# DeepRec-AI/HybridBackend

Measured on AMD Instinct MI355X. Metric: M-lookups/sec, 26-col Criteo-shape dim16, 1/2/4/8 GPUs; % HBM roofline, higher is better.
Workload: dtype f32

## Files before the change

hybridbackend_amd/csrc/lookup_bwd.hip:

```cpp
#include <alloca.h>
#include <stdlib.h>
#include <string.h>

#include <algorithm>
#include <map>
#include <type_traits>
#include <mutex>
#include <vector>

#include "lookup_common.h"

#ifndef HBK_BWD_WAVES
#define HBK_BWD_WAVES 4
#endif

namespace hbk {
size_t det_sort_temp_bytes(size_t n, int end_bit);
int det_sort_pairs(void* temp, size_t temp_bytes, const uint64_t* keys_in, uint64_t* keys_out,
                   const uint32_t* vals_in, uint32_t* vals_out, size_t n, int end_bit,
                   hipStream_t stream);
size_t det_scan_temp_bytes(size_t n);
int det_scan(void* temp, size_t temp_bytes, const int32_t* in, int32_t* out, size_t n,
             hipStream_t stream);
namespace {
// ... 116 lines not shown
  int64_t n_seg;
  int32_t dim;
  int32_t chunks;
  uint8_t lpr_log2, ids64, combiner, vec4;
  int32_t n_buckets;
  int32_t tile0;
  int32_t bucket0;
  int32_t segtile0;
  int32_t split_t;
  int32_t e_max;
  int32_t merge0;
  int32_t scan0;
  int32_t n_runs;
  int32_t grad_stride;
  uint32_t dense_mul;
  int32_t tpitch;
  uint8_t rowsort;
  uint8_t det;
  uint8_t pad_;
  uint8_t packed;
};

struct GArgs {
  int32_t n_cols;
  float lr;
  int32_t apply;
  int32_t xcd;
  int32_t tile0[kMaxCols];
  int32_t bucket0[kMaxCols];
  int32_t merge0[kMaxCols];
  int32_t scan0[kMaxCols];
  int32_t segtile0[kMaxCols];
  int32_t xcd_w;
  int32_t stage_p;
  int32_t xcd_start[10][9];
  GCol col[kMaxCols];
};
static_assert(sizeof(GArgs) <= 24576, "kernarg budget");
static_assert(kMaxCols <= kWave, "one lane per column in HBK_FIND_COL");
static_assert(kSlots <= 65536 && kCP <= 65536, "16-bit LDS indices");

#define HBK_FIND_COL(ARGS, FIELD)                                                  \
  int ci;                                                                          \
  {                                                                                \
    const int l__ = (int)threadIdx.x & (kWave - 1);                                \
    const int v__ = l__ < (ARGS).n_cols ? (ARGS).FIELD[l__] : 0x7fffffff;          \
    ci = (int)__builtin_popcountll(__ballot(v__ <= (int)blockIdx.x)) - 1;          \
    ci = __builtin_amdgcn_readfirstlane(ci);                                       \
  }                                                                                \
  const auto& c = (ARGS).col[ci];

__device__ inline uint32_t mix32(uint64_t row) {
  uint32_t k = (uint32_t)row ^ ((uint32_t)(row >> 32) * 0x9e3779b1u);
  k ^= k >> 16;
  k *= 0x85ebca6bu;
  k ^= k >> 13;
  k *= 0xc2b2ae35u;
  k ^= k >> 16;
  return k;
}

__device__ inline int bucket_of(const GCol& c, uint64_t row) {
  if (c.dense_mul != 0) return (int)__umulhi((uint32_t)row, c.dense_mul);
  return (int)__umulhi(mix32(row), (uint32_t)c.n_buckets);
}

struct RunCursor {
  int k = -1;
  int64_t next = 0;
  int64_t id_delta = 0;
  int64_t grad_delta = 0;
};

__device__ inline void run_seek(const GCol& c, int64_t j, RunCursor& rc) {
  while (j >= rc.next) {
    ++rc.k;
    const int64_t start = c.run_start[rc.k];
    rc.next = rc.k + 1 < c.n_runs ? c.run_start[rc.k + 1] : (int64_t)1 << 62;
    rc.id_delta = c.run_ids[rc.k] - start;
    rc.grad_delta = c.run_grads[rc.k] - start * c.dim;
  }
}

template <typename V>
__device__ inline void scale_segments(const GCol& c, const float* grad, int32_t stride, int combiner,
                                      int64_t s0, int n, const int32_t* sp) {
  constexpr int VE = sizeof(V) / 4;
  constexpr int kU = 4;
  const int tid = (int)threadIdx.x;
  const int sub = tid & ((1 << c.lpr_log2) - 1);
  const int groups = kBlock >> c.lpr_log2;
  if (sub >= c.chunks) return;
  for (int s = tid >> c.lpr_log2; s < n; s += kU * groups) {
    V g[kU];
    int32_t len[kU];
#pragma unroll
    for (int u = 0; u < kU; ++u) {
      const int ss = s + u * groups < n ? s + u * groups : n - 1;
      len[u] = s + u * groups < n ? sp[ss + 1] - sp[ss] : 0;
      g[u] = __builtin_nontemporal_load(reinterpret_cast<const V*>(
          grad + (s0 + ss) * (int64_t)stride + (int64_t)sub * VE));
    }
#pragma unroll
    for (int u = 0; u < kU; ++u) {
      if (len[u] <= 0) continue;
      const V v = combiner == HBK_COMBINER_MEAN ? g[u] / (float)len[u]
                                                : g[u] / sqrtf((float)len[u]);
      *reinterpret_cast<V*>(c.scaled + (s0 + s + u * groups) * (int64_t)c.dim + (int64_t)sub * VE) = v;
    }
  }
}

__device__ inline int32_t seg_search_wave(const int32_t* splits, int64_t n_seg, int32_t j) {
  const int lane = (int)threadIdx.x & (kWave - 1);
  int64_t lo = 0, n = n_seg;
  while (n > 1) {
    const int64_t step = (n + kWave - 1) / kWave;
    const int64_t s = lo + (int64_t)lane * step;
    const bool le = s < lo + n && splits[s] <= j;
    int k = (int)__builtin_popcountll(__ballot(le));
    if (k < 1) k = 1;
    const int64_t nlo = lo + (int64_t)(k - 1) * step;
    const int64_t rest = lo + n - nlo;
    lo = nlo;
    n = rest < step ? rest : step;
  }
  return (int32_t)lo;
}

__device__ inline int32_t tile_segments(const GCol& c, int64_t j_first, int64_t j_last,
                                        int32_t* seg_lds, int32_t* ends) {
  static_assert(kTile == kBlock * kPerThread && kPerThread % 4 == 0, "whole int4 per thread");
  const int tid = (int)threadIdx.x, lane = tid & (kWave - 1), wave = tid >> 6;
  if (wave == 0) {
    const int32_t s = seg_search_wave(c.splits, c.n_seg, (int32_t)j_first);
    if (tid == 0) ends[0] = s;
  } else if (wave == 1) {
    const int32_t s = seg_search_wave(c.splits, c.n_seg, (int32_t)j_last);
    if (tid == kWave) ends[1] = s;
  }
  int4* const v4 = reinterpret_cast<int4*>(seg_lds) + tid * (kPerThread / 4);
#pragma unroll
  for (int q = 0; q < kPerThread / 4; ++q) v4[q] = make_int4(0, 0, 0, 0);
  __syncthreads();
  const int32_t s_lo = ends[0], s_hi = ends[1];
  for (int32_t s = s_lo + 1 + tid; s <= s_hi; s += kBlock) {
    const int64_t p = (int64_t)c.splits[s] - j_first;
    if (p >= 0 && p < kTile) atomicAdd(&seg_lds[p], 1);
  }
  __syncthreads();
  int32_t x[kPerThread];
#pragma unroll
  for (int q = 0; q < kPerThread / 4; ++q) {
    const int4 v = v4[q];
    x[4 * q] = v.x;
    x[4 * q + 1] = v.y;
    x[4 * q + 2] = v.z;
    x[4 * q + 3] = v.w;
  }
#pragma unroll
  for (int q = 1; q < kPerThread; ++q) x[q] += x[q - 1];
  int32_t incl = x[kPerThread - 1];
#pragma unroll
  for (int o = 1; o < kWave; o <<= 1) {
    const int32_t y = __shfl_up(incl, o, kWave);
    if (lane >= o) incl += y;
  }
  if (lane == kWave - 1) ends[2 + wave] = incl;
  __syncthreads();
  int32_t before = incl - x[kPerThread - 1];
  for (int w = 0; w < wave; ++w) before += ends[2 + w];
#pragma unroll
  for (int q = 0; q < kPerThread / 4; ++q) {
    v4[q] = make_int4(x[4 * q] + before, x[4 * q + 1] + before, x[4 * q + 2] + before,
                      x[4 * q + 3] + before);
  }
  __syncthreads();
  return s_lo;
}

__global__ __launch_bounds__(kBlock) void bwd_segof_kernel(const GArgs a) {
  __shared__ int32_t sp[kBlock + 1];
  HBK_FIND_COL(a, segtile0)
  const int64_t s0 = ((int64_t)blockIdx.x - c.segtile0) * kBlock;
  const int tid = (int)threadIdx.x;
  const int n = c.n_seg - s0 < kBlock ? (int)(c.n_seg - s0) : kBlock;
  if (tid < n) sp[tid] = c.splits[s0 + tid];
  if (tid == 0) sp[n] = c.splits[s0 + n];
  __syncthreads();
  const int32_t lo = sp[0], hi = c.seg_of != nullptr ? sp[n] : sp[0];
  for (int32_t j = lo + tid; j < hi; j += kBlock) {
    int s = 0, e = n;
    while (e - s > 1) {
      const int mid = (s + e) >> 1;
      if (sp[mid] <= j) {
        s = mid;
      } else {
        e = mid;
      }
    }
    c.seg_of[j] = (int32_t)(s0 + s);
  }
  if (c.scaled != nullptr) {
    if (c.vec4) {
      scale_segments<f32x4>(c, c.grad_out, c.grad_stride, c.combiner, s0, n, sp);
    } else {
      scale_segments<float>(c, c.grad_out, c.grad_stride, c.combiner, s0, n, sp);
    }
  }
}

template <bool SIMPLE>
__global__ __launch_bounds__(kBlock) void bwd_hist_kernel(const GArgs a) {
  extern __shared__ int32_t counters[];
  HBK_FIND_COL(a, tile0)
  const int P = c.n_buckets;
  const int tid = (int)threadIdx.x;
  const int ctile = (int)blockIdx.x - c.tile0;
  const int64_t base = (int64_t)ctile * kTile;
  RunCursor rc;
  int64_t id[kBatch];
  auto load_batch = [&](int k0) {
#pragma unroll
    for (int k = 0; k < kBatch; ++k) {
      const int64_t j = base + (int64_t)(k0 + k) * kBlock + tid;
      id[k] = 0;
      if (j < c.n_ids) {
        if (!SIMPLE && c.n_runs > 0) run_seek(c, j, rc);
        id[k] = load_id(c.ids, SIMPLE ? 1 : c.ids64, SIMPLE ? j : j + rc.id_delta);
      }
    }
  };
  load_batch(0);
  for (int p = tid; p < P; p += kBlock) counters[p] = 0;
  __syncthreads();
  for (int k0 = 0; k0 < kPerThread; k0 += kBatch) {
    if (k0 > 0) load_batch(k0);
#pragma unroll
    for (int k = 0; k < kBatch; ++k) {
      const int64_t j = base + (int64_t)(k0 + k) * kBlock + tid;
      if (j < c.n_ids) {
        const uint64_t r = id_to_row(c.map, id[k]);
        if (r != kNoRow) atomicAdd(&counters[SIMPLE ? (int)__umulhi((uint32_t)r, c.dense_mul) : bucket_of(c, r)], 1);
      }
    }
  }
  __syncthreads();
  for (int p = tid; p < P; p += kBlock) c.hist[(int64_t)ctile * P + p] = counters[p];
  if (c.scaled != nullptr) {
    __shared__ int32_t sp[kBlock + 1];
    const int64_t n_tiles = (c.n_ids + kTile - 1) / kTile;
    const int64_t per = (c.n_seg + n_tiles - 1) / n_tiles;
    const int64_t s_begin = (int64_t)ctile * per;
    const int64_t s_end = s_begin + per < c.n_seg ? s_begin + per : c.n_seg;
    for (int64_t s0 = s_begin; s0 < s_end; s0 += kBlock) {
      const int n = s_end - s0 < kBlock ? (int)(s_end - s0) : kBlock;
      __syncthreads();
      if (tid < n) sp[tid] = c.splits[s0 + tid];
      if (tid == 0) sp[n] = c.splits[s0 + n];
      __syncthreads();
      if (c.vec4) {
        scale_segments<f32x4>(c, c.raw_grad, c.raw_stride, c.raw_combiner, s0, n, sp);
      } else {
        scale_segments<float>(c, c.raw_grad, c.raw_stride, c.raw_combiner, s0, n, sp);
      }
    }
  }
}

__device__ inline void scan_tiles_of_bucket(const GCol& c, int p) {
  const int P = c.n_buckets;
  const int n_tiles = (int)((c.n_ids + kTile - 1) / kTile);
  int32_t* h = c.hist + p;
  int32_t run = 0;
  int t = 0;
  for (; t + 16 <= n_tiles; t += 16) {
    int32_t x[16];
#pragma unroll
    for (int k = 0; k < 16; ++k) x[k] = h[(int64_t)(t + k) * P];
#pragma unroll
    for (int k = 0; k < 16; ++k) {
      h[(int64_t)(t + k) * P] = run;
      run += x[k];
    }
  }
  for (; t + 4 <= n_tiles; t += 4) {
    int32_t x[4];
#pragma unroll
    for (int k = 0; k < 4; ++k) x[k] = h[(int64_t)(t + k) * P];
#pragma unroll
    for (int k = 0; k < 4; ++k) {
      h[(int64_t)(t + k) * P] = run;
      run += x[k];
    }
  }
  for (; t < n_tiles; ++t) {
    const int32_t x = h[(int64_t)t * P];
    h[(int64_t)t * P] = run;
    run += x;
  }
  c.bstart[p] = run;
}

__global__ __launch_bounds__(kBlock) void bwd_scan_tiles_kernel(const GArgs a) {
  HBK_FIND_COL(a, scan0)
  const int p = ((int)blockIdx.x - c.scan0) * kBlock + (int)threadIdx.x;
  if (p < c.n_buckets) scan_tiles_of_bucket(c, p);
}

__device__ inline void scan_buckets_of_column(const GCol& c, int32_t* wave_tot, int32_t* n_extra_lds) {
  int32_t& n_extra = *n_extra_lds;
  const int P = c.n_buckets;
  const int tid = (int)threadIdx.x, lane = tid & (kWave - 1), wave = tid >> 6;
  const int per = (P + kBlock - 1) / kBlock;
  const int beg = tid * per;
  const int end = beg + per < P ? beg + per : P;
  if (tid == 0) n_extra = 0;
  int32_t sum = 0;
  for (int p = beg; p < end; ++p) sum += c.bstart[p];
  int32_t incl = sum;
#pragma unroll
  for (int off = 1; off < kWave; off <<= 1) {
    const int32_t y = __shfl_up(incl, off, kWave);
    if (lane >= off) incl += y;
  }
  if (lane == kWave - 1) wave_tot[wave] = incl;
  __syncthreads();
  int32_t run = incl - sum;
  for (int w = 0; w < wave; ++w) run += wave_tot[w];
  for (int p = beg; p < end; ++p) {
    const int32_t n_b = c.bstart[p];
    c.bstart[p] = run;
    c.desc[p] = make_int4(run, n_b, p, 0);
    c.pcount[p] = 0;
    if (n_b > c.split_t) {
      const int32_t extras = (n_b - 1) / c.split_t;
      const int32_t base = atomicAdd(&n_extra, extras);
      for (int32_t e = 0; e < extras; ++e) {
        c.work[2 * (base + e)] = p;
        c.work[2 * (base + e) + 1] = e + 1;
        c.desc[P + base + e] = make_int4(run, n_b, p, e + 1);
      }
    }
    run += n_b;
  }
  __syncthreads();
  for (int e = n_extra + tid; e < c.e_max; e += kBlock) c.desc[P + e] = make_int4(0, 0, -1, 0);
  if (tid == kBlock - 1) {
    c.bstart[P] = run;
    c.counter[0] = 0;
    c.counter[1] = 0;
    *c.n_extra = n_extra;
  }
}

__global__ __launch_bounds__(kBlock) void bwd_scan_kernel(const GArgs a) {
  __shared__ int32_t wave_tot[kWavesPerBlock];
  __shared__ int32_t n_extra;
  scan_buckets_of_column(a.col[blockIdx.x], wave_tot, &n_extra);
}

__global__ __launch_bounds__(kBlock) void bwd_scan_fused_kernel(const GArgs a) {
  __shared__ int32_t wave_tot[kWavesPerBlock];
  __shared__ int32_t n_extra;
  const GCol& c = a.col[blockIdx.x];
  for (int p = (int)threadIdx.x; p < c.n_buckets; p += kBlock) scan_tiles_of_bucket(c, p);
  __syncthreads();
  scan_buckets_of_column(c, wave_tot, &n_extra);
}

constexpr int kXcdScatterBit = 30;

__global__ __launch_bounds__(kBlock) void bwd_scatter_pairs_kernel(const GArgs a) {
  extern __shared__ int32_t run[];
  const int blk = xcd_contiguous((int)blockIdx.x, (int)gridDim.x, (a.xcd >> kXcdScatterBit) & 1);
  int ci;
  {
    const int l__ = (int)threadIdx.x & (kWave - 1);
    const int v__ = l__ < a.n_cols ? a.tile0[l__] : 0x7fffffff;
    ci = (int)__builtin_popcountll(__ballot(v__ <= blk)) - 1;
    ci = __builtin_amdgcn_readfirstlane(ci);
  }
  const GCol& c = a.col[ci];
  const int P = c.n_buckets;
  const int tid = (int)threadIdx.x;
  const int ctile = blk - c.tile0;
  const int64_t base = (int64_t)ctile * kTile;
  __shared__ int32_t sp_lds[kTile];
  __shared__ int32_t seg_ends[2 + kWavesPerBlock];
  const bool seg_inline = c.splits != nullptr && c.seg_of == nullptr;
  int32_t s_lo = 0;
  if (seg_inline) {
    const int64_t j_last = (base + kTile < c.n_ids ? base + kTile : c.n_ids) - 1;
    s_lo = tile_segments(c, base, j_last, sp_lds, seg_ends);
  }
  RunCursor rc;
  int64_t id[kBatch];
  int32_t seg[kBatch];
  auto load_batch = [&](int k0) {
#pragma unroll
    for (int k = 0; k < kBatch; ++k) {
      const int64_t j = base + (int64_t)(k0 + k) * kBlock + tid;
      id[k] = 0;
      seg[k] = (int32_t)j;
      if (j < c.n_ids) {
        if (c.n_runs > 0) {
          run_seek(c, j, rc);
          if (!c.det) seg[k] = (int32_t)(uint32_t)(rc.grad_delta + j * c.dim);
        }
        id[k] = load_id(c.ids, c.ids64, j + rc.id_delta);
        if (c.seg_of != nullptr) {
          seg[k] = c.seg_of[j];
        } else if (seg_inline) {
          seg[k] = s_lo + sp_lds[(k0 + k) * kBlock + tid];
        }
      }
    }
  };
  load_batch(0);
  for (int p = tid; p < P; p += kBlock) run[p] = c.bstart[p] + c.hist[(int64_t)ctile * P + p];
  __syncthreads();
  for (int k0 = 0; k0 < kPerThread; k0 += kBatch) {
    if (k0 > 0) load_batch(k0);
#pragma unroll
    for (int k = 0; k < kBatch; ++k) {
      const int64_t j = base + (int64_t)(k0 + k) * kBlock + tid;
      if (j < c.n_ids) {
        const uint64_t r = id_to_row(c.map, id[k]);
        if (r != kNoRow) {
          const int32_t pos = atomicAdd(&run[bucket_of(c, r)], 1);
          if (c.packed) {
            c.pair_row[0][pos] = (int64_t)((r << 32) | (uint64_t)(uint32_t)seg[k]);
          } else {
            c.pair_row[0][pos] = (int64_t)r;
            c.pair_seg[0][pos] = seg[k];
          }
        }
      }
    }
  }
}

constexpr int kStageMaxBuckets = 1024;

template <bool SIMPLE>
__global__ __launch_bounds__(kBlock, 4) void bwd_scatter_staged_kernel(const GArgs a) {
  extern __shared__ int32_t stage_dyn[];
  int32_t* const counters = stage_dyn;
  int32_t* const first = stage_dyn + a.stage_p;
  int32_t* const st_seg = stage_dyn + 2 * a.stage_p;
  __shared__ int64_t st_row[kTile];
  __shared__ uint16_t st_b[SIMPLE ? 1 : kTile];
  __shared__ int32_t wave_cnt[kWavesPerBlock];
  __shared__ int32_t n_staged;
  const int blk = xcd_contiguous((int)blockIdx.x, (int)gridDim.x, (a.xcd >> kXcdScatterBit) & 1);
  int ci;
  {
    const int l__ = (int)threadIdx.x & (kWave - 1);
    const int v__ = l__ < a.n_cols ? a.tile0[l__] : 0x7fffffff;
    ci = (int)__builtin_popcountll(__ballot(v__ <= blk)) - 1;
    ci = __builtin_amdgcn_readfirstlane(ci);
  }
  const GCol& c = a.col[ci];
  const int P = c.n_buckets;
  const int tid = (int)threadIdx.x, lane = tid & (kWave - 1), wave = tid >> 6;
  const int ctile = blk - c.tile0;
  const int64_t base = (int64_t)ctile * kTile;
  __shared__ int32_t seg_ends[2 + kWavesPerBlock];
  int32_t* const sp_lds = reinterpret_cast<int32_t*>(st_row);
  const bool seg_inline = c.splits != nullptr && (SIMPLE || c.seg_of == nullptr);
  RunCursor rc;
  int64_t id[kPerThread];
  int32_t seg[kPerThread];
#pragma unroll
  for (int k = 0; k < kPerThread; ++k) {
    const int64_t j = base + (int64_t)k * kBlock + tid;
    id[k] = 0;
    seg[k] = (int32_t)j;
    if (j < c.n_ids) {
      if (!SIMPLE && c.n_runs > 0) {
        run_seek(c, j, rc);
        if (!c.det) seg[k] = (int32_t)(uint32_t)(rc.grad_delta + j * c.dim);
      }
      id[k] = load_id(c.ids, SIMPLE ? 1 : c.ids64, SIMPLE ? j : j + rc.id_delta);
      if (!SIMPLE && c.seg_of != nullptr) seg[k] = c.seg_of[j];
    }
  }
  const int per = (P + kBlock - 1) / kBlock;
  const int beg = tid * per;
  const int end = beg + per < P ? beg + per : P;
  int32_t gpos[kStageMaxBuckets / kBlock];
#pragma unroll
  for (int q = 0; q < kStageMaxBuckets / kBlock; ++q) {
    const int p = beg + q;
    gpos[q] = q < per && p < end ? c.bstart[p] + c.hist[(int64_t)ctile * P + p] : 0;
  }
  if (seg_inline) {
    const int64_t j_last = (base + kTile < c.n_ids ? base + kTile : c.n_ids) - 1;
    const int32_t s_lo = tile_segments(c, base, j_last, sp_lds, seg_ends);
#pragma unroll
    for (int k = 0; k < kPerThread; ++k) seg[k] = s_lo + sp_lds[k * kBlock + tid];
  }
  for (int p = tid; p < P; p += kBlock) counters[p] = 0;
  __syncthreads();
  int32_t br[kPerThread];
#pragma unroll
  for (int k = 0; k < kPerThread; ++k) {
    const int64_t j = base + (int64_t)k * kBlock + tid;
    br[k] = -1;
    if (j < c.n_ids) {
      const uint64_t r = id_to_row(c.map, id[k]);
      id[k] = (int64_t)r;
      if (r != kNoRow) {
        const int b = SIMPLE ? (int)__umulhi((uint32_t)r, c.dense_mul) : bucket_of(c, r);
        br[k] = b | (atomicAdd(&counters[b], 1) << 10);
      }
    }
  }
  __syncthreads();
  int32_t sum_c = 0;
#pragma unroll
  for (int q = 0; q < kStageMaxBuckets / kBlock; ++q) {
    if (q < per && beg + q < end) sum_c += counters[beg + q];
  }
  int32_t incl_c = sum_c;
#pragma unroll
  for (int off = 1; off < kWave; off <<= 1) {
    const int32_t w = __shfl_up(incl_c, off, kWave);
    if (lane >= off) incl_c += w;
  }
  if (lane == kWave - 1) wave_cnt[wave] = incl_c;
  __syncthreads();
  int32_t run_c = incl_c - sum_c;
  for (int w = 0; w < wave; ++w) run_c += wave_cnt[w];
#pragma unroll
  for (int q = 0; q < kStageMaxBuckets / kBlock; ++q) {
    const int p = beg + q;
    if (q < per && p < end) {
      const int32_t n_c = counters[p];
      first[p] = run_c;
      counters[p] = gpos[q] - run_c;
      run_c += n_c;
    }
  }
  if (tid == kBlock - 1) n_staged = run_c;
  __syncthreads();
#pragma unroll
  for (int k = 0; k < kPerThread; ++k) {
    if (br[k] >= 0) {
      const int b = br[k] & 1023;
      const int L = first[b] + (br[k] >> 10);
      if (SIMPLE || c.packed) {
        st_row[L] = (int64_t)(((uint64_t)id[k] << 32) | (uint64_t)(uint32_t)seg[k]);
      } else {
        st_row[L] = id[k];
        st_seg[L] = seg[k];
      }
      if (!SIMPLE) st_b[L] = (uint16_t)b;
    }
  }
  __syncthreads();
  const int n_st = n_staged;
#pragma unroll
  for (int k = 0; k < kPerThread; ++k) {
    const int L = k * kBlock + tid;
    if (L < n_st) {
      const int sb = SIMPLE ? (int)__umulhi((uint32_t)((uint64_t)st_row[L] >> 32), c.dense_mul) : (int)st_b[L];
      const int32_t pos = counters[sb] + L;
      c.pair_row[0][pos] = st_row[L];
      if (!SIMPLE && !c.packed) c.pair_seg[0][pos] = st_seg[L];
    }
  }
}

#ifdef HBK_BWD_STAMPS
__device__ unsigned long long g_grp_trace[kTraceBlocks * kTraceSlots];
#define HBK_GSTAMP(i)                                                                       \
  do {                                                                                      \
    if (threadIdx.x == 0 && blockIdx.x < kTraceBlocks) {                                    \
      g_grp_trace[blockIdx.x * kTraceSlots + (i)] = __builtin_amdgcn_s_memrealtime();       \
    }                                                                                       \
  } while (0)
#else
#define HBK_GSTAMP(i)
#endif

constexpr int kGroupMaxBuckets = 2 * kBlock;

struct GSync {
  int32_t* hist;
  int32_t* zero;
  int64_t zero_words;
  SyncWait wait;
};

template <bool SIMPLE>
__global__ __launch_bounds__(kBlock, 4) void bwd_group_kernel(const GArgs a, const GSync y) {
  __shared__ int32_t counters[kGroupMaxBuckets];
  __shared__ int32_t tot_s[kGroupMaxBuckets], pre_s[kGroupMaxBuckets];
  __shared__ int64_t st_row[kTile];
  extern __shared__ int32_t st_seg[];
  __shared__ uint16_t st_b[kTile];
  __shared__ int32_t wave_tot[kWavesPerBlock], wave_cnt[kWavesPerBlock];
  __shared__ int32_t n_extra, gave_up, n_staged;
  const int tid = (int)threadIdx.x, lane = tid & (kWave - 1), wave = tid >> 6;
  HBK_GSTAMP(0);
  for (int64_t j = (int64_t)blockIdx.x * kBlock + tid; j < y.zero_words;
       j += (int64_t)gridDim.x * kBlock) {
    y.zero[j] = 0;
  }
// ... 2425 lines not shown
      if (lr != 0.0f) bits |= (uintptr_t)h.table | (uintptr_t)h.accum | ((uintptr_t)(uint32_t)h.table_pitch * 4);
      vec4 = vec4 && h.dim % 4 == 0 && bits % 16 == 0 && h.n_runs == 0;
      ++k;
    }
    if (k == 0) continue;
    for (int q = k; q <= kMaxCols; ++q) a.base[q] = (int32_t)total;
    a.n_cols = k;
    a.row_bits = bits_for(max_rows);
    a.apply = apply;
    a.lr = lr;
    a.total = total;
    const int end_bit = a.row_bits + (k > 1 ? bits_for((uint64_t)k - 1) : 0);
    a.keys = keys;
    a.vals = vals;
    a.heads = heads;
    a.ranks = ranks;
    hipLaunchKernelGGL(det_keys_kernel, dim3((unsigned)tiles), dim3(kBlock), 0, stream, a);
    HBK_HIP_OK(hipGetLastError());
    int rc = det_sort_pairs(ws + l.temp, l.temp_bytes, keys, skeys, vals, svals, (size_t)total, end_bit,
                            stream);
    if (rc != HBK_OK) return rc;
    a.keys = skeys;
    a.vals = svals;
    const unsigned tiles_p = (unsigned)((total + kDetTile - 1) / kDetTile);
    hipLaunchKernelGGL(det_heads_kernel, dim3(tiles_p), dim3(kBlock), 0, stream, a);
    HBK_HIP_OK(hipGetLastError());
    rc = det_scan(ws + l.temp, l.temp_bytes, heads, ranks, (size_t)total, stream);
    if (rc != HBK_OK) return rc;
    if (vec4) {
      det_launch_reduce<f32x4>(a, max_dim / 4, stream);
    } else {
      det_launch_reduce<float>(a, max_dim, stream);
    }
    HBK_HIP_OK(hipGetLastError());
    hipLaunchKernelGGL(det_counts_kernel, dim3(1), dim3(kWave), 0, stream, a);
    HBK_HIP_OK(hipGetLastError());
  }
  return HBK_OK;
}

}
}

#ifdef HBK_BWD_STAMPS
extern "C" int hbk_debug_grp_trace(unsigned long long* out, int reset) {
  using namespace hbk;
  HBK_HIP_OK(hipDeviceSynchronize());
  if (out != nullptr) {
    HBK_HIP_OK(hipMemcpyFromSymbol(out, HIP_SYMBOL(g_grp_trace), sizeof(g_grp_trace)));
  }
  if (reset) {
    static unsigned long long z[kTraceBlocks * kTraceSlots];
    HBK_HIP_OK(hipMemcpyToSymbol(HIP_SYMBOL(g_grp_trace), z, sizeof(z)));
  }
  return HBK_OK;
}
extern "C" int hbk_debug_bwd_sub(unsigned long long* out) {
  using namespace hbk;
  HBK_HIP_OK(hipDeviceSynchronize());
  HBK_HIP_OK(hipMemcpyFromSymbol(out, HIP_SYMBOL(g_bwd_sub), sizeof(g_bwd_sub)));
  return HBK_OK;
}
extern "C" int hbk_debug_bwd_trace(unsigned long long* out, int reset) {
  using namespace hbk;
  HBK_HIP_OK(hipDeviceSynchronize());
  if (out != nullptr) {
    HBK_HIP_OK(hipMemcpyFromSymbol(out, HIP_SYMBOL(g_bwd_trace), sizeof(g_bwd_trace)));
  }
  if (reset) {
    static unsigned long long z[kTraceBlocks * kTraceSlots];
    HBK_HIP_OK(hipMemcpyToSymbol(HIP_SYMBOL(g_bwd_trace), z, sizeof(z)));
  }
  return HBK_OK;
}
#endif

extern "C" size_t hbk_group_lookup_bwd_workspace_bytes(int32_t n_cols,
                                                       const hbk_lookup_grad_column_t* cols) {
  if (n_cols <= 0 || cols == nullptr) return 0;
  if (hbk::any_weighted(n_cols, cols)) {
    std::vector<hbk_lookup_grad_column_t> as_sum;
    const size_t tb = hbk::weighted_as_sum(n_cols, cols, nullptr, &as_sum);
    return tb + hbk_group_lookup_bwd_workspace_bytes(n_cols, as_sum.data());
  }
  std::vector<hbk::ColInfo> info;
  for (int32_t c = 0; c < n_cols; ++c) info.push_back(hbk::col_info(cols[c]));
  return hbk::call_layout(n_cols, cols, info).total;
}

extern "C" int hbk_group_lookup_bwd(int32_t n_cols, const hbk_lookup_grad_column_t* cols,
                                    float apply_lr, void* workspace, size_t workspace_bytes,
                                    hbk_stream_t stream_) {
  return hbk_group_lookup_bwd_apply(n_cols, cols, HBK_APPLY_SGD, apply_lr, workspace,
                                    workspace_bytes, stream_);
}

namespace hbk {
int device_cus() {
  static std::mutex mu;
  static std::map<int, int> cus;
  int dev = 0;
  if (hipGetDevice(&dev) != hipSuccess) return 256;
  std::lock_guard<std::mutex> lock(mu);
  auto it = cus.find(dev);
  if (it != cus.end()) return it->second;
  int n = 0;
  if (hipDeviceGetAttribute(&n, hipDeviceAttributeMultiprocessorCount, dev) != hipSuccess || n <= 0) {
    n = 256;
  }
  cus[dev] = n;
  return n;
}

namespace {
constexpr int kHelperStreams = 4;
struct BwdHelpers {
  hipStream_t s[kHelperStreams];
  hipEvent_t fork, join[kHelperStreams];
  std::mutex mu;
};

BwdHelpers* bwd_helpers(hipStream_t caller) {
  static std::mutex table_mu;
  static std::map<int, BwdHelpers*> table;
  hipStreamCaptureStatus capturing = hipStreamCaptureStatusNone;
  (void)hipStreamIsCapturing(caller, &capturing);
  if (capturing != hipStreamCaptureStatusNone) return nullptr;
  int dev = 0;
  if (hipGetDevice(&dev) != hipSuccess) return nullptr;
  BwdHelpers* h = nullptr;
  {
    std::lock_guard<std::mutex> lock(table_mu);
    auto it = table.find(dev);
    if (it == table.end()) {
      h = new BwdHelpers();
      bool ok = true;
      for (int i = 0; i < kHelperStreams; ++i) {
        ok = ok && hipStreamCreateWithFlags(&h->s[i], hipStreamNonBlocking) == hipSuccess;
        ok = ok && hipEventCreateWithFlags(&h->join[i], hipEventDisableTiming) == hipSuccess;
      }
      ok = ok && hipEventCreateWithFlags(&h->fork, hipEventDisableTiming) == hipSuccess;
      if (!ok) {
        delete h;
        h = nullptr;
      }
      table[dev] = h;
    } else {
      h = it->second;
    }
  }
  return h;
}

int check_columns(int32_t n_cols, const hbk_lookup_grad_column_t* cols, int32_t apply, float apply_lr,
                  std::vector<ColInfo>* info) {
  HBK_REQUIRE(apply == HBK_APPLY_SGD || apply == HBK_APPLY_ADAGRAD,
              "group_lookup_bwd: apply must be HBK_APPLY_SGD or HBK_APPLY_ADAGRAD, got %d", apply);
  HBK_REQUIRE(n_cols >= 0, "group_lookup_bwd: n_cols must be >= 0, got %d", n_cols);
  if (n_cols == 0) return HBK_OK;
  HBK_REQUIRE(cols != nullptr, "group_lookup_bwd: cols is NULL");
  for (int32_t c = 0; c < n_cols; ++c) {
    const hbk_lookup_grad_column_t& h = cols[c];
    HBK_REQUIRE(h.dim >= 1, "group_lookup_bwd: column %d: dim must be >= 1", c);
    HBK_REQUIRE(h.rows >= 0 && h.n_ids >= 0 && h.n_segments >= 0,
                "group_lookup_bwd: column %d: negative size", c);
    HBK_REQUIRE(h.n_ids < (1ll << 30), "group_lookup_bwd: column %d: more than 2^30-1 ids", c);
    HBK_REQUIRE(h.ids_dtype == HBK_INT32 || h.ids_dtype == HBK_INT64,
                "group_lookup_bwd: column %d: ids must be int32 or int64", c);
    HBK_REQUIRE(h.bucket >= 0 && h.divisor >= 1,
                "group_lookup_bwd: column %d: bad bucket/divisor", c);
    HBK_REQUIRE(h.combiner >= HBK_COMBINER_SUM && h.combiner <= HBK_COMBINER_SQRTN,
                "group_lookup_bwd: column %d: unknown combiner %d", c, h.combiner);
    HBK_REQUIRE(h.row_splits != nullptr || h.n_segments == h.n_ids,
                "group_lookup_bwd: column %d: n_segments must equal n_ids when row_splits "
                "is NULL", c);
    HBK_REQUIRE(h.n_unique != nullptr, "group_lookup_bwd: column %d: n_unique is NULL", c);
    HBK_REQUIRE(h.n_ids == 0 || (h.ids && h.grad_out), "group_lookup_bwd: column %d: NULL buffer", c);
    HBK_REQUIRE(h.n_ids == 0 || (h.unique_rows != nullptr) == (h.grad_rows != nullptr),
                "group_lookup_bwd: column %d: unique_rows and grad_rows go together", c);
    HBK_REQUIRE(h.n_ids == 0 || h.grad_rows != nullptr || apply_lr != 0.0f,
                "group_lookup_bwd: column %d: no output buffers and no optimizer step: nothing "
                "to do (unique_rows / grad_rows may only be NULL with apply_lr != 0)", c);
    HBK_REQUIRE(apply_lr == 0.0f || h.table != nullptr || h.n_ids == 0,
                "group_lookup_bwd: column %d: table is NULL but apply_lr != 0", c);
    HBK_REQUIRE(apply_lr == 0.0f || apply != HBK_APPLY_ADAGRAD || h.accum != nullptr ||
                    h.n_ids == 0,
                "group_lookup_bwd: column %d: Adagrad needs the accumulator table", c);
    HBK_REQUIRE(h.table_pitch == 0 || h.table_pitch >= h.dim,
                "group_lookup_bwd: column %d: table_pitch %d is smaller than dim %d", c, h.table_pitch,
                h.dim);
    HBK_REQUIRE((h.flags & ~HBK_GRAD_DETERMINISTIC) == 0, "group_lookup_bwd: column %d: unknown flags 0x%x", c,
                (unsigned)h.flags);
    HBK_REQUIRE(h.n_runs >= 0, "group_lookup_bwd: column %d: n_runs must be >= 0", c);
    HBK_REQUIRE(h.n_runs == 0 || (h.row_splits == nullptr && h.run_start && h.run_ids &&
                                  h.run_grads),
                "group_lookup_bwd: column %d: segmented inputs need run tables and no "
                "row_splits", c);
    HBK_REQUIRE(h.id_weights == nullptr || h.n_runs == 0,
                "group_lookup_bwd: column %d: id_weights cannot be combined with segmented inputs "
                "(run_*: the owner-side reduce is never weighted)", c);
  }
  return check_layouts(n_cols, cols, apply_lr, info);
}

std::vector<int32_t> order_columns(int32_t n_cols, const hbk_lookup_grad_column_t* cols,
                                   const std::vector<ColInfo>& info, int form) {
  std::vector<int32_t> order;
  for (int pass = 0; pass < 2; ++pass) {
    for (int32_t c = 0; c < n_cols; ++c) {
      const ColInfo& ci = info[(size_t)c];
      if (cols[c].n_ids <= 0 || ci.form != form) continue;
      if ((pass == 0) == (ci.onepass != (options().bwd_large_first != 0))) order.push_back(c);
    }
  }
  return order;
}

int32_t next_group(const std::vector<ColInfo>& info, const std::vector<int32_t>& order, int32_t* q0,
                   int group_cols, int32_t* members) {
  const bool group_onepass = info[(size_t)order[(size_t)*q0]].onepass;
  int32_t k_n = 0;
  while (*q0 < (int32_t)order.size() && k_n < group_cols &&
         info[(size_t)order[(size_t)*q0]].onepass == group_onepass) {
    members[k_n++] = order[(size_t)(*q0)++];
  }
  std::stable_sort(members, members + k_n,
                   [&](int32_t a, int32_t b) { return info[(size_t)a].kind < info[(size_t)b].kind; });
  return k_n;
}

struct Carve {
  char* counter;
  char* desc;
  char* buf;
};
template <typename T>
inline T* buf_at(char* base, size_t off) {
  return off == kNoBuf ? nullptr : reinterpret_cast<T*>(base + off);
}
inline float* rows_at(char* base, size_t off) {
  return off == kNoBuf ? nullptr : reinterpret_cast<float*>(((uintptr_t)(base + off) + 15) & ~(uintptr_t)15);
}

struct KindCol { int32_t n_buckets, e_max, weight; };
struct Group {
  GArgs args, seg_args;
  bool onepass;
  int32_t k = 0, ks = 0;
  int64_t tiles = 0, buckets = 0, segtiles = 0, merges = 0, scans = 0, sync_words = 0;
  size_t lds_hist = 0;
  bool small_scan = true;
  int64_t slot_lo[kKinds] = {0}, slot_hi[kKinds] = {0};
  int64_t merge_lo[kKinds] = {0}, merge_hi[kKinds] = {0};
  bool have_kind[kKinds] = {false};
  std::vector<KindCol> kind_cols[kKinds];
  int64_t xcd_grid[kKinds] = {0};
};

int add_column(Group& g, const hbk_lookup_grad_column_t& h, const ColInfo& ci, bool det, Carve* at) {
  const ColPlan& p = ci.p;
  const ColLayout& l = ci.lay;
  const int32_t k = g.k;
  GCol& d = g.args.col[k];
  memset(&d, 0, sizeof(d));
  d.ids = h.ids;
  d.grad_out = h.grad_out;
  d.splits = h.row_splits;
  d.unique_rows = h.unique_rows;
  d.grad_rows = h.grad_rows;
  d.n_unique = h.n_unique;
  d.counter = reinterpret_cast<int32_t*>(at->counter);
  at->counter += 256;
  d.desc = reinterpret_cast<int4*>(at->desc);
  at->desc += l.desc_bytes;
  char* const base = at->buf;
  at->buf += l.bytes;
  d.table = h.table;
  d.accum = h.accum;
  d.hist = buf_at<int32_t>(base, l.hist);
  d.bstart = buf_at<int32_t>(base, l.bstart);
  d.pair_row[0] = buf_at<int64_t>(base, l.pair_row);
  d.pair_seg[0] = buf_at<int32_t>(base, l.pair_seg);
  d.packed = l.pair_seg == kNoBuf ? 1 : 0;
  d.seg_of = buf_at<int32_t>(base, l.seg_of);
  float* const scaled = rows_at(base, l.scaled);
  d.work = buf_at<int32_t>(base, l.work);
  d.n_extra = buf_at<int32_t>(base, l.n_extra);
  d.pcount = buf_at<int32_t>(base, l.pcount);
  d.part_rows = buf_at<int64_t>(base, l.part_rows);
  d.part_vals = rows_at(base, l.part_vals);
  if (h.grad_rows == nullptr) {
    d.no_emit = 1;
    d.unique_rows = buf_at<int64_t>(base, l.step_rows);
    d.grad_rows = rows_at(base, l.step_vals);
  }
  d.split_t = p.split_t;
  d.e_max = p.e_max;
  d.dense_mul = p.dense_mul;
  d.rowsort = p.rowsort ? 1 : 0;
  d.det = det ? 1 : 0;
  d.merge0 = (int32_t)g.merges;
  const int64_t merge_blocks = p.e_max < kMergeBlocks ? p.e_max : kMergeBlocks;
  d.scan0 = (int32_t)g.scans;
  g.scans += ((int64_t)p.n_buckets + kBlock - 1) / kBlock;
  g.small_scan = g.small_scan && p.n_buckets <= 4 * kBlock && p.tiles <= 64;
  d.sync0 = (int32_t)g.sync_words;
  g.sync_words += (int64_t)p.tiles * p.n_buckets;
  d.run_start = h.run_start;
  d.run_ids = h.run_ids;
  d.run_grads = h.run_grads;
  d.n_runs = h.n_runs;
  d.grad_stride = h.grad_stride > 0 ? h.grad_stride : h.dim;
  d.map = make_idmap(h.bucket, h.divisor, h.rows);
  d.n_ids = h.n_ids;
  d.n_seg = h.n_segments;
  d.dim = h.dim;
  d.tpitch = h.table_pitch > 0 ? h.table_pitch : h.dim;
  d.chunks = ci.shape.chunks;
  d.lpr_log2 = ci.shape.lpr_log2;
  d.vec4 = ci.shape.vec4;
  d.ids64 = h.ids_dtype == HBK_INT64;
  d.combiner = (uint8_t)h.combiner;
  d.n_buckets = p.n_buckets;
  d.tile0 = (int32_t)g.tiles;
  d.bucket0 = (int32_t)g.buckets;
  if (!g.have_kind[ci.kind]) {
    g.have_kind[ci.kind] = true;
    g.slot_lo[ci.kind] = g.buckets;
    g.merge_lo[ci.kind] = g.merges;
  }
  g.kind_cols[ci.kind].push_back({p.n_buckets, p.e_max, 24 + h.dim});
  g.tiles += p.tiles;
  g.buckets += (int64_t)p.n_buckets + p.e_max;
  g.merges += merge_blocks;
  g.slot_hi[ci.kind] = g.buckets;
  g.merge_hi[ci.kind] = g.merges;
  if (g.tiles >= (1ll << 31) || g.buckets >= (1ll << 31)) {
    return fail(HBK_INVALID_ARGUMENT, "group_lookup_bwd: grid too large");
  }
  if ((size_t)4 * p.n_buckets > g.lds_hist) g.lds_hist = (size_t)4 * p.n_buckets;
  g.args.tile0[k] = d.tile0;
  g.args.bucket0[k] = d.bucket0;
  g.args.merge0[k] = d.merge0;
  g.args.scan0[k] = d.scan0;
  g.args.segtile0[k] = 0;
  const bool scale_in_hist = scaled != nullptr && d.seg_of == nullptr && !g.onepass &&
                             options().bwd_scale_fused != 0 && h.n_segments > 0;
  if (scale_in_hist) {
    d.scaled = scaled;
    d.raw_grad = h.grad_out;
    d.raw_stride = h.grad_stride > 0 ? h.grad_stride : h.dim;
    d.raw_combiner = h.combiner;
  }
  if (!scale_in_hist && h.row_splits != nullptr && h.n_segments > 0 &&
      (d.seg_of != nullptr || scaled != nullptr)) {
    GCol& sdesc = g.seg_args.col[g.ks];
    sdesc = d;
    sdesc.scaled = scaled;
    sdesc.segtile0 = (int32_t)g.segtiles;
    g.seg_args.segtile0[g.ks] = (int32_t)g.segtiles;
    g.segtiles += (h.n_segments + kBlock - 1) / kBlock;
    ++g.ks;
  }
  if (scaled != nullptr && h.n_segments > 0) {
    d.grad_out = scaled;
    d.grad_stride = h.dim;
    d.combiner = HBK_COMBINER_SUM;
  }
  ++g.k;
  return HBK_OK;
}

void trace_group(const Group& g, const hbk_lookup_grad_column_t* cols, const std::vector<ColInfo>& info,
                 const int32_t* members, int group_no, int stream_no) {
  int64_t g_ids = 0, g_bytes = 0;
  int by_kind[kKinds] = {0};
  for (int32_t i = 0; i < g.k; ++i) {
    g_ids += cols[members[i]].n_ids;
    g_bytes += (int64_t)cols[members[i]].n_ids * cols[members[i]].dim * 4;
    ++by_kind[info[(size_t)members[i]].kind];
  }
  fprintf(stderr, "[hbk bwd] group %d on stream %d: %d columns (%s), %lld ids, %.1f MB of gradient rows, "
          "%lld tiles, %lld job slots; columns by kind", group_no, stream_no, g.k,
          g.onepass ? "one-launch" : "large", (long long)g_ids, (double)g_bytes / 1e6, (long long)g.tiles,
          (long long)g.buckets);
  for (int q = 0; q < kKinds; ++q) {
    if (by_kind[q] != 0) fprintf(stderr, " %d:%d", q, by_kind[q]);
  }
  fprintf(stderr, "\n");
}

void place_xcds(Group& g) {
  GArgs& args = g.args;
  args.xcd = 0;
  for (int kind = 0; kind < kKinds; ++kind) {
    if (!g.have_kind[kind] || options().bwd_xcd == 0) continue;
    bool even = options().bwd_xcd == 2;
    if (!even) {
      const int64_t per = slots_per_block(kind);
      const int64_t n = (g.slot_hi[kind] - g.slot_lo[kind] + per - 1) / per;
      const int64_t q = n / 8, r = n % 8;
      double work[8] = {0}, total = 0;
      int64_t slot = 0;
      int x = 0;
      int64_t x_end = (r > 0 ? q + 1 : q) * per;
      for (const KindCol& kc : g.kind_cols[kind]) {
        for (int part = 0; part < 2; ++part) {
          int64_t len = part == 0 ? kc.n_buckets : kc.e_max;
          const double w = part == 0 ? (double)kc.weight : 0.0;
          while (len > 0) {
            while (x < 7 && slot >= x_end) {
              ++x;
              x_end += (x < r ? q + 1 : q) * per;
            }
            const int64_t take = x < 7 && x_end - slot < len ? x_end - slot : len;
            work[x] += w * (double)take;
            total += w * (double)take;
            slot += take;
            len -= take;
          }
        }
      }
      double heaviest = 0;
      for (double w : work) heaviest = w > heaviest ? w : heaviest;
      even = total > 0 && heaviest <= 1.08 * total / 8;
    }
    if (even) args.xcd |= 1 << kind;
  }
  args.xcd_w = 0;
  if ((options().bwd_xcd == 4 || options().bwd_xcd == 1 || options().bwd_xcd == 3) && kTeams == 1) {
    for (int kind = 0; kind < kKinds; ++kind) {
      if (!g.have_kind[kind]) continue;
      if (options().bwd_xcd != 4 && !((args.xcd >> kind) & 1)) continue;
      double total = 0;
      for (const KindCol& kc : g.kind_cols[kind]) total += (double)kc.weight * kc.n_buckets;
      if (total <= 0) continue;
      int32_t* st = args.xcd_start[kind];
      st[0] = 0;
      int x = 1;
      double acc = 0;
      int64_t slot = 0;
      for (const KindCol& kc : g.kind_cols[kind]) {
        for (int64_t b = 0; b < kc.n_buckets; ++b) {
          while (x < 8 && acc >= total * x / 8) st[x++] = (int32_t)(slot + b);
          acc += kc.weight;
        }
        slot += (int64_t)kc.n_buckets + kc.e_max;
      }
      while (x <= 8) st[x++] = (int32_t)slot;
      st[8] = (int32_t)(g.slot_hi[kind] - g.slot_lo[kind]);
      int64_t longest = 0;
      for (int q = 0; q < 8; ++q) longest = st[q + 1] - st[q] > longest ? st[q + 1] - st[q] : longest;
      g.xcd_grid[kind] = 8 * longest;
      args.xcd_w |= 1 << kind;
    }
  }
  if (options().bwd_xcd == 1 || options().bwd_xcd == 2) args.xcd |= 1 << kXcdScatterBit;
}

bool launch_grouping(Group& g, hipStream_t ls, hipStream_t caller, GSync* sync) {
  GArgs& args = g.args;
  const int32_t k = g.k;
  const dim3 tiles((unsigned)g.tiles), block(kBlock);
  if (g.ks > 0) {
    g.seg_args.n_cols = g.ks;
    g.seg_args.lr = 0.f;
    hipLaunchKernelGGL(bwd_segof_kernel, dim3((unsigned)g.segtiles), block, 0, ls, g.seg_args);
  }
  bool simple_group = options().bwd_simple != 0;
  bool unpacked = false;
  for (int32_t i = 0; i < k; ++i) {
    const GCol& c = args.col[i];
    simple_group = simple_group && c.n_runs == 0 && c.seg_of == nullptr && c.packed != 0 && c.ids64 != 0 &&
                   c.dense_mul != 0;
    unpacked = unpacked || c.packed == 0;
  }
  const size_t lds_tail = (unpacked ? (size_t)kTile * 4 : 0) + (size_t)options().bwd_lds_pad * 1024;
  memset(sync, 0, sizeof(*sync));
  const auto group_kernel = simple_group ? &bwd_group_kernel<true> : &bwd_group_kernel<false>;
  bool onepass = g.onepass && g.sync_words < (1ll << 30);
  if (onepass) {
    SyncTake take;
    onepass = sync_take(ls, (size_t)g.sync_words, &take, reinterpret_cast<const void*>(group_kernel), kBlock,
                        64, caller);
    if (onepass) {
      sync->hist = take.words;
      sync->zero = take.zero;
      sync->zero_words = take.zero_words;
      sync->wait = sync_wait_of(take);
    }
  }
  if (onepass) {
    SyncChain chain(ls);
    hipLaunchKernelGGL(group_kernel, tiles, block, lds_tail, ls, args, *sync);
    return true;
  }
  hipLaunchKernelGGL(simple_group ? &bwd_hist_kernel<true> : &bwd_hist_kernel<false>, tiles, block, g.lds_hist,
                     ls, args);
  if (g.small_scan) {
    hipLaunchKernelGGL(bwd_scan_fused_kernel, dim3((unsigned)k), block, 0, ls, args);
  } else {
    hipLaunchKernelGGL(bwd_scan_tiles_kernel, dim3((unsigned)g.scans), block, 0, ls, args);
    hipLaunchKernelGGL(bwd_scan_kernel, dim3((unsigned)k), block, 0, ls, args);
  }
  if (g.lds_hist <= (size_t)4 * kStageMaxBuckets && options().bwd_scatter_staged != 0) {
    args.stage_p = (int32_t)(g.lds_hist / 4);
    hipLaunchKernelGGL(simple_group ? &bwd_scatter_staged_kernel<true> : &bwd_scatter_staged_kernel<false>,
                       tiles, block, 2 * g.lds_hist + lds_tail, ls, args);
  } else {
    hipLaunchKernelGGL(bwd_scatter_pairs_kernel, tiles, block, g.lds_hist, ls, args);
  }
  return false;
}

int launch_reduce_merge(const Group& g, bool det, int32_t apply, float apply_lr, const int4* desc,
                        const int32_t* poison, hipStream_t ls) {
  const GArgs& args = g.args;
  const int step = apply_lr == 0.0f ? 0 : apply == HBK_APPLY_ADAGRAD ? 2 : 1;
  typedef void (*reduce_fn)(const GArgs, const int4*, int, int, const int32_t*);
  typedef void (*merge_fn)(const GArgs, int, const int32_t*);
#define HBK_BY_STEP(K, V, ...) {&K<V, 0, ##__VA_ARGS__>, &K<V, 1, ##__VA_ARGS__>, &K<V, 2, ##__VA_ARGS__>}
  static const reduce_fn kReduce[kKinds][3] = {
      HBK_BY_STEP(bwd_dense_kernel, f32x4, false), HBK_BY_STEP(bwd_dense_kernel, float, false),
      HBK_BY_STEP(bwd_dense_kernel, f32x4, true), HBK_BY_STEP(bwd_dense_kernel, float, true),
      HBK_BY_STEP(bwd_reduce_kernel, f32x4, false), HBK_BY_STEP(bwd_reduce_kernel, float, false),
      {nullptr, &bwd_reduce_kernel<f32x4, 1, true>, &bwd_reduce_kernel<f32x4, 2, true>},
      {nullptr, &bwd_reduce_kernel<float, 1, true>, &bwd_reduce_kernel<float, 2, true>},
      HBK_BY_STEP(bwd_rowsort_kernel, f32x4), HBK_BY_STEP(bwd_rowsort_kernel, float)};
  static const merge_fn kMerge[kKinds][3] = {
      HBK_BY_STEP(bwd_dense_merge_kernel, f32x4), HBK_BY_STEP(bwd_dense_merge_kernel, float),
      HBK_BY_STEP(bwd_dense_merge_kernel, f32x4), HBK_BY_STEP(bwd_dense_merge_kernel, float),
      HBK_BY_STEP(bwd_merge_kernel, f32x4, false), HBK_BY_STEP(bwd_merge_kernel, float, false),
      {nullptr, &bwd_merge_kernel<f32x4, 1, true>, &bwd_merge_kernel<f32x4, 2, true>},
      {nullptr, &bwd_merge_kernel<float, 1, true>, &bwd_merge_kernel<float, 2, true>},
      HBK_BY_STEP(bwd_rowsort_merge_kernel, f32x4), HBK_BY_STEP(bwd_rowsort_merge_kernel, float)};
  static const reduce_fn kReduceDet[2][3] = {HBK_BY_STEP(bwd_rowsort_kernel, f32x4, true),
                                             HBK_BY_STEP(bwd_rowsort_kernel, float, true)};
#undef HBK_BY_STEP
  int status = HBK_OK;
  if (det) {
    hipLaunchKernelGGL(bwd_rowsort_count_kernel, dim3((unsigned)g.buckets), dim3(kBlock), 0, ls, args, desc,
                       (int)g.buckets, poison);
  }
  for (int kind = 0; kind < kKinds; ++kind) {
    if (!g.have_kind[kind]) continue;
    const int64_t n_slots = g.slot_hi[kind] - g.slot_lo[kind];
    const int64_t per = slots_per_block(kind);
    const int64_t grid = g.xcd_grid[kind] > 0 ? g.xcd_grid[kind] : (n_slots + per - 1) / per;
    if (det && bucket_kind_of(kind) != kRowSorted) {
      status = fail(HBK_INTERNAL, "group_lookup_bwd: a deterministic column without row-sorted buckets");
      break;
    }
    hipLaunchKernelGGL(det ? kReduceDet[kind & 1][step] : kReduce[kind][step],
                       dim3((unsigned)grid), dim3(kBlock), 0, ls, args, desc, (int)g.slot_lo[kind],
                       (int)g.slot_hi[kind], poison);
  }
  for (int kind = 0; kind < kKinds; ++kind) {
    if (!g.have_kind[kind]) continue;
    hipLaunchKernelGGL(kMerge[kind][step], dim3((unsigned)(g.merge_hi[kind] - g.merge_lo[kind])),
                       dim3(kBlock), 0, ls, args, (int)g.merge_lo[kind], poison);
  }
  const hipError_t launch_err = hipGetLastError();
  if (launch_err != hipSuccess) {
    status = fail(HBK_INTERNAL, "group_lookup_bwd: launch failed: %s", hipGetErrorString(launch_err));
  }
  return status;
}

int bwd_planned(int32_t n_cols, const hbk_lookup_grad_column_t* cols, const std::vector<ColInfo>& info,
                int form, int32_t apply, float apply_lr, void* workspace, hipStream_t stream) {
  const bool det = form == kFormInOrder;
  const std::vector<int32_t> order = order_columns(n_cols, cols, info, form);
  const int32_t live_cols = (int32_t)order.size();
  Carve at;
  at.counter = reinterpret_cast<char*>(((uintptr_t)workspace + 255) & ~(uintptr_t)255);
  at.desc = at.counter + (size_t)256 * order.size();
  at.buf = at.desc;
  for (int32_t c : order) at.buf += info[(size_t)c].lay.desc_bytes;
  for (int32_t c = 0; c < n_cols; ++c) {
    if (cols[c].n_ids == 0 && info[(size_t)c].form == form) {
      HBK_HIP_OK(hipMemsetAsync(cols[c].n_unique, 0, sizeof(int32_t), stream));
    }
  }

  int group_cols = options().bwd_group_cols;
  if (group_cols <= 0 || group_cols > kMaxCols) group_cols = kMaxCols;
  bool mixed = false;
  for (int32_t q = 1; q < live_cols; ++q) {
    mixed = mixed || info[(size_t)order[q]].onepass != info[(size_t)order[0]].onepass;
  }
  const int n_streams = options().bwd_streams < 0 ? 0 : options().bwd_streams > kHelperStreams
                                                           ? kHelperStreams : options().bwd_streams;
  BwdHelpers* helpers = (live_cols > group_cols || mixed) && n_streams > 0 ? bwd_helpers(stream) : nullptr;
  std::unique_lock<std::mutex> hold;
  if (helpers != nullptr) {
    hold = std::unique_lock<std::mutex>(helpers->mu);
    HBK_HIP_OK(hipEventRecord(helpers->fork, stream));
    for (int i = 0; i < kHelperStreams; ++i) {
      HBK_HIP_OK(hipStreamWaitEvent(helpers->s[i], helpers->fork, 0));
    }
  }
  int status = HBK_OK;
  int group_no = 0;
  int32_t q0 = 0;
  while (q0 < live_cols && status == HBK_OK) {
    const int stream_no = helpers != nullptr ? group_no % n_streams : -1;
    hipStream_t ls = helpers != nullptr ? helpers->s[stream_no] : stream;
// ... 164 lines not shown
```

Measured before the change: 30000.

## Parallelize per-bucket tile scan across rows of threads with shared-memory partials

The tile-histogram exclusive scan used to give one thread per bucket, which walked all tiles serially. Now each block handles 32 buckets and splits the tile range across kBlock/32 thread rows. Each row sums its segment, combines the row partials through shared memory, and writes back offsets, holding values in registers when the segment is small. This adds more blocks and a barrier, and re-reads the histogram when segments are long.

```diff
diff --git a/hybridbackend_amd/csrc/lookup_bwd.hip b/hybridbackend_amd/csrc/lookup_bwd.hip
--- a/hybridbackend_amd/csrc/lookup_bwd.hip
+++ b/hybridbackend_amd/csrc/lookup_bwd.hip
@@ -442,10 +442,71 @@
   c.bstart[p] = run;
 }
 
+constexpr int kScanLanes = 32;
+constexpr int kScanRows = kBlock / kScanLanes;
+constexpr int kScanHeld = 256 / kScanRows;
+
 __global__ __launch_bounds__(kBlock) void bwd_scan_tiles_kernel(const GArgs a) {
-  HBK_FIND_COL(a, scan0)
-  const int p = ((int)blockIdx.x - c.scan0) * kBlock + (int)threadIdx.x;
-  if (p < c.n_buckets) scan_tiles_of_bucket(c, p);
+  __shared__ int32_t part[kScanRows][kScanLanes];
+  const int blk = xcd_contiguous((int)blockIdx.x, (int)gridDim.x, 1);
+  int ci;
+  {
+    const int l__ = (int)threadIdx.x & (kWave - 1);
+    const int v__ = l__ < a.n_cols ? a.scan0[l__] : 0x7fffffff;
+    ci = (int)__builtin_popcountll(__ballot(v__ <= blk)) - 1;
+    ci = __builtin_amdgcn_readfirstlane(ci);
+  }
+  const GCol& c = a.col[ci];
+  const int P = c.n_buckets;
+  const int lane = (int)threadIdx.x % kScanLanes, row = (int)threadIdx.x / kScanLanes;
+  const int p = (blk - c.scan0) * kScanLanes + lane;
+  const bool live = p < P;
+  const int n_tiles = (int)((c.n_ids + kTile - 1) / kTile);
+  const int per = (n_tiles + kScanRows - 1) / kScanRows;
+  const int t0 = row * per < n_tiles ? row * per : n_tiles;
+  const int t1 = t0 + per < n_tiles ? t0 + per : n_tiles;
+  int32_t* const h = c.hist + (live ? p : 0);
+  const bool held = per <= kScanHeld;
+  int32_t x[kScanHeld];
+  int32_t sum = 0;
+  if (held) {
+#pragma unroll
+    for (int k = 0; k < kScanHeld; ++k) x[k] = live && t0 + k < t1 ? h[(int64_t)(t0 + k) * P] : 0;
+#pragma unroll
+    for (int k = 0; k < kScanHeld; ++k) sum += x[k];
+  } else if (live) {
+    for (int t = t0; t < t1; t += 16) {
+      int32_t y[16];
+#pragma unroll
+      for (int k = 0; k < 16; ++k) y[k] = t + k < t1 ? h[(int64_t)(t + k) * P] : 0;
+#pragma unroll
+      for (int k = 0; k < 16; ++k) sum += y[k];
+    }
+  }
+  part[row][lane] = sum;
+  __syncthreads();
+  int32_t run = 0;
+  for (int r = 0; r < row; ++r) run += part[r][lane];
+  if (!live) return;
+  if (held) {
+#pragma unroll
+    for (int k = 0; k < kScanHeld; ++k) {
+      if (t0 + k < t1) h[(int64_t)(t0 + k) * P] = run;
+      run += x[k];
+    }
+  } else {
+    for (int t = t0; t < t1; t += 16) {
+      int32_t y[16];
+#pragma unroll
+      for (int k = 0; k < 16; ++k) y[k] = t + k < t1 ? h[(int64_t)(t + k) * P] : 0;
+#pragma unroll
+      for (int k = 0; k < 16; ++k) {
+        if (t + k < t1) h[(int64_t)(t + k) * P] = run;
+        run += y[k];
+      }
+    }
+  }
+  if (row == kScanRows - 1) c.bstart[p] = run;
 }
 
 __device__ inline void scan_buckets_of_column(const GCol& c, int32_t* wave_tot, int32_t* n_extra_lds) {
@@ -3477,7 +3538,7 @@
   d.merge0 = (int32_t)g.merges;
   const int64_t merge_blocks = p.e_max < kMergeBlocks ? p.e_max : kMergeBlocks;
   d.scan0 = (int32_t)g.scans;
-  g.scans += ((int64_t)p.n_buckets + kBlock - 1) / kBlock;
+  g.scans += ((int64_t)p.n_buckets + kScanLanes - 1) / kScanLanes;
   g.small_scan = g.small_scan && p.n_buckets <= 4 * kBlock && p.tiles <= 64;
   d.sync0 = (int32_t)g.sync_words;
   g.sync_words += (int64_t)p.tiles * p.n_buckets;
```

After: 29970. No clear change (-0.1%).
